# Parsoa/SVDSS

Hardware: AMD Instinct MI355X
Metric: reads/sec through search+call, 30x HiFi 15 kb reads vs 3 Gb ref, 1/2/4/8 GPU (higher is better)
Workload: dtype int64

## Files before the change

include/svdss_hip.h:

```cpp
#ifndef SVDSS_HIP_H
#define SVDSS_HIP_H

#include <stdint.h>

#ifdef __cplusplus
extern "C" {
#endif

#define SVDSS_OK 0
#define SVDSS_EINVAL 1
#define SVDSS_ENOMEM 2
#define SVDSS_EIO 3
#define SVDSS_EHIP 4
#define SVDSS_ENODEV 5
#define SVDSS_ERANGE 6

const char* svdss_strerror(int code);
const char* svdss_last_hip_error(void);

int svdss_nt6_encode(const char* seq, int64_t n, uint8_t* out);

typedef struct svdss_index svdss_index_t;

int svdss_index_build(const uint8_t* contigs, const int64_t* lens, int32_t n_contigs,
// ... 326 lines not shown
int32_t svdss_ref_stream_tile_bytes(void);

int svdss_place_sfs_batch(svdss_ref_t* ref, const int32_t* tid, const int32_t* pos, const uint32_t* cigar,
                          const int64_t* cigar_off, const int32_t* sfs_qs, const int32_t* sfs_len, const int64_t* sfs_off,
                          int64_t n_aln, int32_t* out_count, int32_t* out, int64_t stats[4]);

int svdss_smooth_batch(svdss_ref_t* ref, const int32_t* tid, const int32_t* pos, const uint32_t* cigar,
                       const int64_t* cigar_off, const uint8_t* seq4, const int64_t* seq4_off, const uint8_t* qual,
                       const int64_t* qual_off, const int32_t* l_seq, const int64_t* cap_off, int64_t n,
                       uint8_t* out_seq4, uint8_t* out_qual, uint32_t* out_cigar, int32_t* out_ncig, int32_t* out_len,
                       int64_t* out_match_mismatch, uint8_t* out_ignore);

typedef struct svdss_aln_batch svdss_aln_batch_t;

int svdss_align_global_batch(const uint8_t* queries, const int64_t* q_off, const uint8_t* targets,
                             const int64_t* t_off, int64_t n_pairs, int32_t m, const int8_t* mat,
                             int32_t gapo, int32_t gape, int32_t gapo2, int32_t gape2, int32_t device,
                             svdss_aln_batch_t** out);
int64_t svdss_aln_batch_npairs(const svdss_aln_batch_t* b);
int64_t svdss_aln_batch_total_cigar(const svdss_aln_batch_t* b);
int64_t svdss_aln_batch_cells(const svdss_aln_batch_t* b);
double svdss_aln_batch_kernel_ms(const svdss_aln_batch_t* b);
int svdss_aln_batch_launch_info(const svdss_aln_batch_t* b, int64_t out[4]);
int svdss_aln_batch_fetch(const svdss_aln_batch_t* b, int32_t* scores, int64_t* n_cigar, uint32_t* cigar);
void svdss_aln_batch_free(svdss_aln_batch_t* b);

typedef struct svdss_poa_batch svdss_poa_batch_t;

int svdss_poa_consensus_batch(const uint8_t* seqs, const int64_t* seq_off, const int64_t* cluster_off,
                              int64_t n_clusters, int32_t device, svdss_poa_batch_t** out);
int64_t svdss_poa_batch_nclusters(const svdss_poa_batch_t* b);
int64_t svdss_poa_batch_total(const svdss_poa_batch_t* b);
int64_t svdss_poa_batch_cells(const svdss_poa_batch_t* b);
double svdss_poa_batch_kernel_ms(const svdss_poa_batch_t* b);
int64_t svdss_poa_batch_hbm(const svdss_poa_batch_t* b);
int64_t svdss_poa_batch_quad_back(const svdss_poa_batch_t* b);
int svdss_poa_quad_selftest(const int32_t* in, int32_t* out, int32_t device);
int svdss_poa_batch_fetch(const svdss_poa_batch_t* b, int64_t* cons_len, uint8_t* cons);
void svdss_poa_batch_free(svdss_poa_batch_t* b);

int svdss_indel_ratio_batch(const uint8_t* a, const int64_t* a_off, const uint8_t* b, const int64_t* b_off,
                            int64_t n_pairs, int32_t device, double* ratio_out, int64_t* lcs_out);
int32_t svdss_indel_ratio_last_kernel(void);

int svdss_call_side_stat(int32_t device, int64_t out[4]);

// ... 41 lines not shown
```

svdss_amd/_lib.py:

```python
import ctypes as C
import os

_HERE = os.path.dirname(os.path.abspath(__file__))
LIB_PATH = os.environ.get("SVDSS_LIB") or os.path.join(_HERE, "libsvdss_hip.so")

SVDSS_OK = 0
SVDSS_SFS_ASSEMBLE = 1
SVDSS_BAM_PUTATIVE = 0x100


class SvdssError(RuntimeError):
    def __init__(self, code, where):
        self.code = code
        msg = lib.svdss_strerror(code).decode()
        hip = lib.svdss_last_hip_error().decode()
        super().__init__(f"{where}: {msg} (code {code})" + (f" [{hip}]" if hip else ""))


def _load():
    if not os.path.exists(LIB_PATH):
        raise ImportError(
            f"{LIB_PATH} not found: build it with `python -c 'import __graft_entry__ as g; g.build()'` "
            "or `make -C svdss_amd/csrc` (hipcc, gfx950). There is no CPU fallback."
        )
# ... 136 lines not shown
    "svdss_fastx_tile_bytes": (_i32, []),
    "svdss_ref_upload": (C.c_int, [_p, _p, _i32, _i32, C.POINTER(_p)]),
    "svdss_ref_upload_parts": (C.c_int, [_p, _p, _i32, _i32, C.POINTER(_p)]),
    "svdss_ref_free": (None, [_p]),
    "svdss_ref_read": (C.c_int, [_p, _pi32, _p, _p]),
    "svdss_ref_stream_create": (C.c_int, [_i32, _i64, C.POINTER(_p)]),
    "svdss_ref_stream_batch": (C.c_int, [_p, _i64, _i32, _i32, _p, _p, _p, _p, _p, _p, _i64]),
    "svdss_ref_stream_result": (C.c_int, [_p, _p]),
    "svdss_ref_stream_download": (C.c_int, [_p, _i64, _p]),
    "svdss_ref_stream_finish": (C.c_int, [_p, _p, _i32, _i32, C.POINTER(_p)]),
    "svdss_ref_stream_drop_host": (None, [_p]),
    "svdss_ref_stream_free": (None, [_p]),
    "svdss_ref_stream_error": (C.c_char_p, [_p]),
    "svdss_ref_stream_tile_bytes": (_i32, []),
    "svdss_place_sfs_batch": (C.c_int, [_p, _p, _p, _p, _p, _p, _p, _p, _i64, _p, _p, _p]),
    "svdss_smooth_batch": (C.c_int, [_p] * 11 + [_i64] + [_p] * 7),
    "svdss_align_global_batch": (C.c_int, [_p, _p, _p, _p, _i64, _i32, _p, _i32, _i32, _i32, _i32, _i32,
                                           C.POINTER(_p)]),
    "svdss_aln_batch_npairs": (_i64, [_p]),
    "svdss_aln_batch_total_cigar": (_i64, [_p]),
    "svdss_aln_batch_cells": (_i64, [_p]),
    "svdss_aln_batch_kernel_ms": (C.c_double, [_p]),
    "svdss_aln_batch_launch_info": (C.c_int, [_p, _p]),
    "svdss_aln_batch_fetch": (C.c_int, [_p, _p, _p, _p]),
    "svdss_aln_batch_free": (None, [_p]),
    "svdss_poa_consensus_batch": (C.c_int, [_p, _p, _p, _i64, _i32, C.POINTER(_p)]),
    "svdss_poa_batch_nclusters": (_i64, [_p]),
    "svdss_poa_batch_total": (_i64, [_p]),
    "svdss_poa_batch_cells": (_i64, [_p]),
    "svdss_poa_batch_kernel_ms": (C.c_double, [_p]),
    "svdss_poa_batch_hbm": (_i64, [_p]),
    "svdss_poa_batch_quad_back": (_i64, [_p]),
    "svdss_poa_quad_selftest": (C.c_int, [_p, _p, C.c_int32]),
    "svdss_poa_batch_fetch": (C.c_int, [_p, _p, _p]),
    "svdss_poa_batch_free": (None, [_p]),
    "svdss_indel_ratio_batch": (C.c_int, [_p, _p, _p, _p, _i64, _i32, _p, _p]),
    "svdss_indel_ratio_last_kernel": (_i32, []),
    "svdss_call_side_stat": (C.c_int, [_i32, _p]),
    "svdss_gzip_stream_create": (C.c_int, [_i32, _i64, C.POINTER(_p)]),
    "svdss_gzip_stream_run": (C.c_int, [_p, _p, _i64, _i32, _pi64]),
    "svdss_gzip_stream_result": (C.c_int, [_p, _p]),
    "svdss_gzip_stream_host_tail": (C.c_int, [_p, _p, _i64]),
    "svdss_gzip_stream_error": (C.c_char_p, [_p]),
    "svdss_gzip_stream_free": (None, [_p]),
}

# ... 10 lines not shown
```

svdss_amd/csrc/call_dp.hip:

```cpp
#include <hip/hip_runtime.h>

#include <cstdint>
#include <algorithm>
#include <chrono>
#include <cstdio>
#include <cstring>
#include <new>
#include <string>
#include <vector>

#include "../../include/svdss_hip.h"
#include "call_streams.h"
#include "dev_arena.h"
#include "hip_check.h"

#define DP_NEG (-0x20000000)
#define DP_THREADS 256

struct GapModel { int q, e, q2, e2; };

__device__ __forceinline__ int dp_gap(int l, const GapModel& g) {
  const int a = g.q + l * g.e, b = g.q2 + l * g.e2;
  return a < b ? a : b;
}

struct AlnPair {
  int64_t q_off, t_off;
  int64_t bnd_off;
  int64_t dir_off;
  int64_t cig_off;
  int32_t ql, tl;
  int32_t slot;
  int32_t waves;
};

__device__ __forceinline__ int dp_shr1(int x) {
  return __builtin_amdgcn_update_dpp(x, x, 0x138, 0xf, 0xf, false);
}

template <int W>
__global__ void __launch_bounds__(64 * W) align_wave_kernel(
    const AlnPair* pairs, const uint8_t* qsyms, const uint8_t* tsyms, int m, const int8_t* mat_g,
    GapModel gm, int32_t* ws, uint8_t* dirs, uint32_t* cigars, int32_t* scores, int32_t* n_cigar, int32_t* abort_flag) {
  const AlnPair P = pairs[blockIdx.x];
  const int ql = P.ql, tl = P.tl;
  const int lane = threadIdx.x & 63, wave = threadIdx.x >> 6;
  const int Wp = W > 1 ? P.waves : 1, NB = Wp + 1;
  if (wave >= Wp) return;
  if (ql <= 0 || tl <= 0) {
    if (lane == 0) { scores[P.slot] = 0; n_cigar[P.slot] = 0; }
    return;
  }
  __shared__ volatile int32_t prog[W + 1];
  __shared__ int32_t s_score;
  const uint8_t* q = qsyms + P.q_off;
  const uint8_t* t = tsyms + P.t_off;
  uint8_t* dir = dirs + P.dir_off;
  const int bstride = ql + 64;
  int32_t* bnd = ws + P.bnd_off;
  {
    int32_t* b0 = bnd + (int64_t)(NB - 1) * 3 * bstride;
    for (int j = threadIdx.x; j < ql; j += 64 * Wp) { b0[j] = -dp_gap(j + 1, gm); b0[bstride + j] = DP_NEG; b0[2 * bstride + j] = DP_NEG; }
    if ((int)threadIdx.x < NB) prog[threadIdx.x] = (int)threadIdx.x == NB - 1 ? ql : 0;
    __builtin_amdgcn_fence(__ATOMIC_RELEASE, "workgroup");
  }
  __syncthreads();
  const int n_stripes = (tl + 63) >> 6;
  int32_t final_score = 0;
  bool aborted = false;
  for (int s = wave; s < n_stripes && !aborted; s += Wp) {
    const int in_slot = (s + NB - 1) % NB, out_slot = s % NB;
    const int32_t* bin = bnd + (int64_t)in_slot * 3 * bstride;
    int32_t* bout = bnd + (int64_t)out_slot * 3 * bstride;
    if (W > 1 && lane == 0) prog[out_slot] = (s + 1) << 20;
    const int i = (s << 6) + lane;
    const bool row_ok = i < tl;
    const int rows = tl - (s << 6) < 64 ? tl - (s << 6) : 64;
    const bool writes_bnd = lane == 63 && s + 1 < n_stripes;
    uint64_t rowbits = 0;
    {
      const int ti = row_ok ? t[i] : 0;
      for (int k = 0; k < m; ++k) rowbits |= (uint64_t)(uint8_t)mat_g[ti * m + k] << (8 * k);
    }
    int32_t Hl = -dp_gap(i + 1, gm), Fl = DP_NEG, F2l = DP_NEG;
    int32_t Hout = 0, Eout = DP_NEG, E2out = DP_NEG;
    int32_t Hd = 0;
    int qcur = 0;
    const int n_steps = ql + rows - 1;
    int32_t nH = 0, nE = 0, nE2 = 0;
    int nq = 0;
    auto fetch = [&](int tau0) {
      const int jj = tau0 + lane;
      const bool in = jj < ql;
      nq = in ? q[jj] : 0;
      if (W > 1 && Wp > 1) {
        const int need = tau0 + 64 < ql ? tau0 + 64 : ql;
        int polls = 0;
        for (;;) {
          const int32_t v = prog[in_slot];
          if ((v >> 20) == s && (v & 0xFFFFF) >= need) break;
          if (++polls > (1 << 22)) { aborted = true; break; }
          __builtin_amdgcn_s_sleep(2);
        }
        if (aborted) { nH = 0; nE = 0; nE2 = 0; return; }
        __builtin_amdgcn_fence(__ATOMIC_ACQUIRE, "workgroup");
        nH = in ? __hip_atomic_load(&bin[jj], __ATOMIC_RELAXED, __HIP_MEMORY_SCOPE_WORKGROUP) : 0;
        nE = in ? __hip_atomic_load(&bin[bstride + jj], __ATOMIC_RELAXED, __HIP_MEMORY_SCOPE_WORKGROUP) : 0;
        nE2 = in ? __hip_atomic_load(&bin[2 * bstride + jj], __ATOMIC_RELAXED, __HIP_MEMORY_SCOPE_WORKGROUP) : 0;
      } else {
        nH = in ? bin[jj] : 0; nE = in ? bin[bstride + jj] : 0; nE2 = in ? bin[2 * bstride + jj] : 0;
      }
    };
    fetch(0);
    uint8_t* dcell = dir + (int64_t)(s << 6) * tl + i;
    for (int tau0 = 0; tau0 < n_steps && !aborted; tau0 += 64) {
      asm volatile("" : "+v"(nq), "+v"(nH), "+v"(nE), "+v"(nE2));
      const int qblk = nq;
      const int32_t bH = nH, bE = nE, bE2 = nE2;
      if (tau0 + 64 < n_steps) fetch(tau0 + 64);
      const int kmax = n_steps - tau0 < 64 ? n_steps - tau0 : 64;
      for (int k = 0; k < kmax; ++k) {
        const int tau = tau0 + k;
        const int qs = __builtin_amdgcn_readlane(qblk, k);
        const int32_t hb = __builtin_amdgcn_readlane(bH, k), eb = __builtin_amdgcn_readlane(bE, k),
                      e2b = __builtin_amdgcn_readlane(bE2, k);
        qcur = dp_shr1(qcur);
        int32_t Hu = dp_shr1(Hout), Eu = dp_shr1(Eout), E2u = dp_shr1(E2out);
        if (lane == 0) { qcur = qs; Hu = hb; Eu = eb; E2u = e2b; }
        const int j = tau - lane;
        if (row_ok && j >= 0 && j < ql) {
          const int32_t hdiag = j == 0 ? (i == 0 ? 0 : -dp_gap(i, gm)) : Hd;
          const int32_t Ein = (Hu - gm.q > Eu ? Hu - gm.q : Eu) - gm.e;
          const int32_t E2in = (Hu - gm.q2 > E2u ? Hu - gm.q2 : E2u) - gm.e2;
          const int32_t Fin = (Hl - gm.q > Fl ? Hl - gm.q : Fl) - gm.e;
          const int32_t F2in = (Hl - gm.q2 > F2l ? Hl - gm.q2 : F2l) - gm.e2;
          int32_t z = hdiag + (int32_t)(int8_t)(rowbits >> (8 * qcur));
          uint32_t d = 0;
          if (Ein > z) { d = 1; z = Ein; }
          if (Fin > z) { d = 2; z = Fin; }
          if (E2in > z) { d = 3; z = E2in; }
          if (F2in > z) { d = 4; z = F2in; }
          if (Ein > z - gm.q) d |= 0x08;
          if (Fin > z - gm.q) d |= 0x10;
          if (E2in > z - gm.q2) d |= 0x20;
          if (F2in > z - gm.q2) d |= 0x40;
          *dcell = (uint8_t)d;
          Hout = z; Eout = Ein; E2out = E2in;
          Hl = z; Fl = Fin; F2l = F2in;
          if (writes_bnd) { bout[j] = z; bout[bstride + j] = Ein; bout[2 * bstride + j] = E2in; }
          if (i == tl - 1 && j == ql - 1) final_score = z;
        }
        Hd = Hu;
        dcell += tl;
      }
      if (W > 1 && Wp > 1 && s + 1 < n_stripes) {
        __builtin_amdgcn_fence(__ATOMIC_RELEASE, "workgroup");
        const int done = tau0 + kmax - 63;
        if (lane == 63) prog[out_slot] = ((s + 1) << 20) | (done < 0 ? 0 : done > ql ? ql : done);
      }
    }
    if (W == 1 || Wp == 1) __syncthreads();
    else if (s + 1 < n_stripes) { __builtin_amdgcn_fence(__ATOMIC_RELEASE, "workgroup"); if (lane == 63) prog[out_slot] = ((s + 1) << 20) | ql; }
    if (s == n_stripes - 1) {
      const int owner = (tl - 1) & 63;
      final_score = __builtin_amdgcn_readlane(final_score, owner);
      if (lane == 0) s_score = final_score;
    }
  }
  if (aborted && lane == 0) atomicExch(abort_flag, 1);
  __syncthreads();
  if (wave != 0) return;
  final_score = s_score;
  {
    if (lane == 0) scores[P.slot] = final_score;
    uint32_t* cg = cigars + P.cig_off;
    int n = 0, i = tl - 1, j = ql - 1, state = 0;
    uint32_t cur_op = 0xffffffffu, cur_len = 0;
    auto push = [&](uint32_t op, uint32_t len) {
      if (op == cur_op) { cur_len += len; return; }
      if (cur_op != 0xffffffffu) { if (lane == 0) cg[n] = (cur_len << 4) | cur_op; ++n; }
      cur_op = op; cur_len = len;
    };
    int i0 = -(1 << 28), j0 = 0;
    uint32_t win = 0;
    while (i >= 0 && j >= 0) {
      int k = i0 - i, d = j - (j0 - k);
      if (k < 0 || k > 63 || d < 0 || d > 3) {
        i0 = i; j0 = j - 1; k = 0; d = 1;
        const int ii = i0 - lane;
        const int64_t jj = (int64_t)j0 - lane;
        win = 0;
        if (ii >= 0) {
#pragma unroll
          for (int x = 0; x < 4; ++x) {
            const int64_t c = jj + x;
            if (c >= 0 && c < ql) win |= (uint32_t)dir[(int64_t)(ii + c) * tl + ii] << (8 * x);
          }
        }
        asm volatile("" : "+v"(win));
      }
      const uint32_t tmp = ((uint32_t)__builtin_amdgcn_readlane((int)win, k) >> (8 * d)) & 0xffu;
      if (state == 0) state = tmp & 7;
      else if (!((tmp >> (state + 2)) & 1)) state = 0;
      if (state == 0) state = tmp & 7;
      if (state == 0) { push(0, 1); --i; --j; }
      else if (state == 1 || state == 3) { push(2, 1); --i; }
      else { push(1, 1); --j; }
    }
    if (i >= 0) push(2, (uint32_t)(i + 1));
    if (j >= 0) push(1, (uint32_t)(j + 1));
    if (cur_op != 0xffffffffu) { if (lane == 0) cg[n] = (cur_len << 4) | cur_op; ++n; }
    if (lane == 0) n_cigar[P.slot] = n;
  }
}

__device__ __forceinline__ void dp_lds_barrier() {
  __builtin_amdgcn_fence(__ATOMIC_RELEASE, "workgroup", "local");
  __builtin_amdgcn_s_barrier();
  __builtin_amdgcn_fence(__ATOMIC_ACQUIRE, "workgroup", "local");
}

struct LcsPair {
  int64_t a_off, b_off, ws_off;
  int32_t la, lb;
};

template <bool LDS>
__global__ void __launch_bounds__(DP_THREADS) lcs_ratio_kernel(const LcsPair* pairs, const uint8_t* as,
                                                              const uint8_t* bs, int32_t* ws,
                                                              int64_t* lcs_out, double* ratio_out) {
  extern __shared__ int32_t dp_lds[];
  const LcsPair P = pairs[blockIdx.x];
  const int la = P.la, lb = P.lb;
  int64_t lcs = 0;
  if (la > 0 && lb > 0) {
    const uint8_t* a = as + P.a_off;
// ... 79 lines not shown
    const int valid = m - 64 * lane;
    const unsigned long long vm = valid >= 64 ? ~0ull : valid <= 0 ? 0ull : ((1ull << valid) - 1);
    int z = (int)__popcll(~V & vm);
    for (int o = 32; o > 0; o >>= 1) z += __shfl_xor(z, o, 64);
    lcs = z;
  }
  if (lane == 0) {
    const int64_t maximum = (int64_t)P.la + P.lb;
    const int64_t dist = maximum - 2 * lcs;
    const double norm_dist = maximum ? (double)dist / (double)maximum : 0.0;
    const double norm_sim = 1.0 - norm_dist;
    lcs_out[blockIdx.x] = lcs;
    ratio_out[blockIdx.x] = norm_sim * 100.0;
  }
}


struct svdss_aln_batch {
  int64_t n_pairs = 0;
  int64_t total_cigar = 0;
  int64_t cells = 0;
  double kernel_ms = 0.0;
  int64_t info[4] = {0, 0, 0, 0};
  std::vector<int32_t> scores;
  std::vector<int64_t> n_cigar;
  std::vector<uint32_t> cigar;
  int device = -1;
  DevArena arena;
};

namespace {
struct DevMem {
  void* p = nullptr;
  ~DevMem() { if (p) (void)hipFree(p); }
  int alloc(size_t bytes) {
    HIPCHK(hipMalloc(&p, bytes ? bytes : 16));
    return SVDSS_OK;
  }
};
}

extern "C" int svdss_align_global_batch(const uint8_t* queries, const int64_t* q_off,
                                        const uint8_t* targets, const int64_t* t_off, int64_t n_pairs,
                                        int32_t m, const int8_t* mat, int32_t gapo, int32_t gape,
                                        int32_t gapo2, int32_t gape2, int32_t device,
                                        svdss_aln_batch_t** out) {
  if (!out || n_pairs < 0 || m < 1 || m > 8 || !mat || device < 0) return SVDSS_EINVAL;
  if (n_pairs > 0 && (!queries || !q_off || !targets || !t_off)) return SVDSS_EINVAL;
  HIPCHK(hipSetDevice(device));
  svdss_aln_batch* b = *out ? *out : new (std::nothrow) svdss_aln_batch();
  if (!b) return SVDSS_ENOMEM;
  *out = b;
  b->n_pairs = n_pairs;
  b->total_cigar = 0;
  b->cells = 0;
  b->kernel_ms = 0.0;
  b->info[0] = b->info[1] = b->info[2] = b->info[3] = 0;
  b->scores.assign((size_t)n_pairs, 0);
  b->n_cigar.assign((size_t)n_pairs, 0);
  b->cigar.clear();
  if (n_pairs == 0) return SVDSS_OK;
  for (int64_t i = 0; i < n_pairs; ++i) {
    const int64_t ql = q_off[i + 1] - q_off[i], tl = t_off[i + 1] - t_off[i];
    if (ql < 0 || tl < 0) return SVDSS_EINVAL;
    if (ql >= (1 << 28) || tl >= (1 << 28)) return SVDSS_ERANGE;
  }
  const int64_t qtot = q_off[n_pairs] - q_off[0], ttot = t_off[n_pairs] - t_off[0];
  if (b->device != device) {
    b->arena.drop();
    b->device = device;
  }
  CallStreamLease lease;
  HIPCHK(lease.acquire(device));
  const hipStream_t st = lease.get();
  const GapModel gm{gapo, gape, gapo2, gape2};
  hipEvent_t ev0, ev1;
  HIPCHK(hipEventCreate(&ev0));
  HIPCHK(hipEventCreate(&ev1));
  int64_t dir_budget = (int64_t)24 << 30;
  {
    size_t free_b = 0, total_b = 0;
    if (hipMemGetInfo(&free_b, &total_b) == hipSuccess)
      dir_budget = std::min<int64_t>(dir_budget, (int64_t)((free_b + b->arena.cap) / 2));
    if (dir_budget < ((int64_t)1 << 30)) dir_budget = (int64_t)1 << 30;
    if (getenv("SVDSS_ALIGN_DIR_MB") && atoll(getenv("SVDSS_ALIGN_DIR_MB")) > 0) dir_budget = atoll(getenv("SVDSS_ALIGN_DIR_MB")) << 20;
  }
  std::vector<int32_t> h_nc((size_t)n_pairs, 0);
  std::vector<std::pair<int64_t, int64_t>> cig_at((size_t)n_pairs);
  std::vector<std::vector<uint32_t>> chunk_cigs;
  int64_t start = 0;
  const int ALN_W = getenv("SVDSS_ALIGN_WAVES") && atoi(getenv("SVDSS_ALIGN_WAVES")) == 8 ? 8 : 4;
  const int64_t aln_frac = getenv("SVDSS_ALIGN_FRAC") && atoll(getenv("SVDSS_ALIGN_FRAC")) > 0 ? atoll(getenv("SVDSS_ALIGN_FRAC")) : 8;
  int64_t max_cells = 0;
  for (int64_t i = 0; i < n_pairs; ++i) max_cells = std::max(max_cells, (q_off[i + 1] - q_off[i]) * (t_off[i + 1] - t_off[i]));
  bool multi = !(getenv("SVDSS_ALIGN_WAVES") && atoi(getenv("SVDSS_ALIGN_WAVES")) <= 1);
  auto waves_of = [&](int64_t ql, int64_t tl) {
    if (!multi || tl < 8 * 64 || ql >= (1 << 20)) return 1;
    return (ql * tl * aln_frac >= max_cells || n_pairs < 2048) ? ALN_W : 1;
  };
  while (start < n_pairs) {
    std::vector<AlnPair> hp;
    int64_t ws = 0, dirb = 0, cig = 0, end = start;
    bool any_multi = false;
    while (end < n_pairs) {
      const int64_t ql = q_off[end + 1] - q_off[end], tl = t_off[end + 1] - t_off[end];
      const int64_t need = (ql + tl) * tl;
      if (end > start && dirb + need > dir_budget) break;
      AlnPair a;
      memset(&a, 0, sizeof a);
      a.q_off = q_off[end] - q_off[0];
      a.t_off = t_off[end] - t_off[0];
      a.bnd_off = ws;
      a.dir_off = dirb;
      a.cig_off = cig;
      a.ql = (int32_t)ql;
      a.tl = (int32_t)tl;
      a.slot = (int32_t)(end - start);
      a.waves = waves_of(ql, tl);
      any_multi = any_multi || a.waves > 1;
      hp.push_back(a);
      cig_at[(size_t)end] = {cig, (int64_t)chunk_cigs.size()};
      ws += 3 * (a.waves + 1) * (ql + 64);
      dirb += need;
      cig += ql + tl + 2;
      b->cells += ql * tl;
      ++end;
    }
    const int64_t np = end - start;
    std::stable_sort(hp.begin(), hp.end(), [](const AlnPair& x, const AlnPair& y) {
      return (int64_t)x.ql * x.tl > (int64_t)y.ql * y.tl;
    });
    const size_t need_bytes = DevArena::padded((size_t)qtot) + DevArena::padded((size_t)ttot) + DevArena::padded(64) +
                              DevArena::padded(sizeof(AlnPair) * (size_t)np) + DevArena::padded(sizeof(int32_t) * (size_t)ws) +
                              DevArena::padded((size_t)dirb) + DevArena::padded(sizeof(uint32_t) * (size_t)cig) +
                              2 * DevArena::padded(sizeof(int32_t) * (size_t)np) + DevArena::padded(64);
    HIPCHK(b->arena.reserve(need_bytes));
    void* d_q = b->arena.take((size_t)qtot);
    void* d_t = b->arena.take((size_t)ttot);
    void* d_mat = b->arena.take(64);
    void* d_pairs = b->arena.take(sizeof(AlnPair) * (size_t)np);
    void* d_ws = b->arena.take(sizeof(int32_t) * (size_t)ws);
    void* d_dir = b->arena.take((size_t)dirb);
    void* d_cig = b->arena.take(sizeof(uint32_t) * (size_t)cig);
    void* d_sc = b->arena.take(sizeof(int32_t) * (size_t)np);
    void* d_nc = b->arena.take(sizeof(int32_t) * (size_t)np);
    void* d_abort = b->arena.take(64);
    if (qtot) HIPCHK(hipMemcpyAsync(d_q, queries + q_off[0], (size_t)qtot, hipMemcpyHostToDevice, st));
    if (ttot) HIPCHK(hipMemcpyAsync(d_t, targets + t_off[0], (size_t)ttot, hipMemcpyHostToDevice, st));
    HIPCHK(hipMemcpyAsync(d_mat, mat, (size_t)(m * m), hipMemcpyHostToDevice, st));
    HIPCHK(hipMemcpyAsync(d_pairs, hp.data(), sizeof(AlnPair) * (size_t)np, hipMemcpyHostToDevice, st));
    HIPCHK(hipMemsetAsync(d_abort, 0, 64, st));
    HIPCHK(hipEventRecord(ev0, st));
    if (any_multi && ALN_W == 8)
      hipLaunchKernelGGL(align_wave_kernel<8>, dim3((unsigned)np), dim3(64 * 8), 0, st, (const AlnPair*)d_pairs,
                         (const uint8_t*)d_q, (const uint8_t*)d_t, (int)m, (const int8_t*)d_mat, gm, (int32_t*)d_ws,
                         (uint8_t*)d_dir, (uint32_t*)d_cig, (int32_t*)d_sc, (int32_t*)d_nc, (int32_t*)d_abort);
    else if (any_multi)
      hipLaunchKernelGGL(align_wave_kernel<4>, dim3((unsigned)np), dim3(64 * 4), 0, st, (const AlnPair*)d_pairs,
                         (const uint8_t*)d_q, (const uint8_t*)d_t, (int)m, (const int8_t*)d_mat, gm, (int32_t*)d_ws,
                         (uint8_t*)d_dir, (uint32_t*)d_cig, (int32_t*)d_sc, (int32_t*)d_nc, (int32_t*)d_abort);
    else
      hipLaunchKernelGGL(align_wave_kernel<1>, dim3((unsigned)np), dim3(64), 0, st, (const AlnPair*)d_pairs,
                         (const uint8_t*)d_q, (const uint8_t*)d_t, (int)m, (const int8_t*)d_mat, gm, (int32_t*)d_ws,
                         (uint8_t*)d_dir, (uint32_t*)d_cig, (int32_t*)d_sc, (int32_t*)d_nc, (int32_t*)d_abort);
    HIPCHK(hipGetLastError());
    HIPCHK(hipEventRecord(ev1, st));
    if (any_multi) {
      int32_t ab = 0;
      HIPCHK(hipMemcpyAsync(&ab, d_abort, sizeof ab, hipMemcpyDeviceToHost, st));
      HIPCHK(hipStreamSynchronize(st));
      if (ab) {
        fprintf(stderr, "[svdss] realignment: a multi-wavefront pair did not finish; the batch runs again with one wavefront per pair\n");
        multi = false;
        ++b->info[3];
        b->cells -= [&] { int64_t c = 0; for (const AlnPair& a : hp) c += (int64_t)a.ql * a.tl; return c; }();
        for (int64_t k = start; k < end; ++k) cig_at[(size_t)k] = {0, 0};
        continue;
      }
    }
    ++b->info[0];
    for (const AlnPair& a : hp) b->info[1] += a.waves > 1;
    b->info[2] = std::max<int64_t>(b->info[2], any_multi ? ALN_W : 1);
    chunk_cigs.emplace_back((size_t)cig);
    HIPCHK(hipMemcpyAsync(&b->scores[(size_t)start], d_sc, sizeof(int32_t) * (size_t)np, hipMemcpyDeviceToHost, st));
    HIPCHK(hipMemcpyAsync(&h_nc[(size_t)start], d_nc, sizeof(int32_t) * (size_t)np, hipMemcpyDeviceToHost, st));
    if (cig) HIPCHK(hipMemcpyAsync(chunk_cigs.back().data(), d_cig, sizeof(uint32_t) * (size_t)cig, hipMemcpyDeviceToHost, st));
    HIPCHK(hipStreamSynchronize(st));
    float ms = 0.f;
    HIPCHK(hipEventElapsedTime(&ms, ev0, ev1));
    b->kernel_ms += ms;
    start = end;
  }
  {
    int64_t total = 0;
    for (int64_t k = 0; k < n_pairs; ++k) total += h_nc[(size_t)k];
    b->cigar.resize((size_t)total);
    int64_t o = 0;
    for (int64_t k = 0; k < n_pairs; ++k) {
      const int32_t nc = h_nc[(size_t)k];
      b->n_cigar[(size_t)k] = nc;
      const uint32_t* src = chunk_cigs[(size_t)cig_at[(size_t)k].second].data() + cig_at[(size_t)k].first;
      for (int x = nc - 1; x >= 0; --x) b->cigar[(size_t)o++] = src[x];
    }
  }
  (void)hipEventDestroy(ev0);
  (void)hipEventDestroy(ev1);
  b->total_cigar = (int64_t)b->cigar.size();
  return SVDSS_OK;
}

extern "C" int64_t svdss_aln_batch_npairs(const svdss_aln_batch_t* b) { return b ? b->n_pairs : -1; }
extern "C" int64_t svdss_aln_batch_total_cigar(const svdss_aln_batch_t* b) { return b ? b->total_cigar : -1; }
extern "C" int64_t svdss_aln_batch_cells(const svdss_aln_batch_t* b) { return b ? b->cells : -1; }
extern "C" double svdss_aln_batch_kernel_ms(const svdss_aln_batch_t* b) { return b ? b->kernel_ms : -1.0; }

extern "C" int svdss_aln_batch_launch_info(const svdss_aln_batch_t* b, int64_t out[4]) {
  if (!b || !out) return SVDSS_EINVAL;
  memcpy(out, b->info, sizeof b->info);
  return SVDSS_OK;
}

extern "C" int svdss_aln_batch_fetch(const svdss_aln_batch_t* b, int32_t* scores, int64_t* n_cigar,
                                     uint32_t* cigar) {
  if (!b) return SVDSS_EINVAL;
  if (scores) memcpy(scores, b->scores.data(), sizeof(int32_t) * b->scores.size());
  if (n_cigar) memcpy(n_cigar, b->n_cigar.data(), sizeof(int64_t) * b->n_cigar.size());
  if (cigar) memcpy(cigar, b->cigar.data(), sizeof(uint32_t) * b->cigar.size());
  return SVDSS_OK;
}

extern "C" void svdss_aln_batch_free(svdss_aln_batch_t* b) { delete b; }

static thread_local int32_t g_ratio_last_kernel = -1;
extern "C" int32_t svdss_indel_ratio_last_kernel(void) { return g_ratio_last_kernel; }

extern "C" int svdss_indel_ratio_batch(const uint8_t* a, const int64_t* a_off, const uint8_t* bsy,
                                       const int64_t* b_off, int64_t n_pairs, int32_t device,
                                       double* ratio_out, int64_t* lcs_out) {
  if (n_pairs < 0 || device < 0) return SVDSS_EINVAL;
  if (n_pairs == 0) return SVDSS_OK;
  if (!a || !a_off || !bsy || !b_off || !ratio_out) return SVDSS_EINVAL;
// ... 91 lines not shown
```

Measured before the change: 8.414 million.

## Add provable score-bound banding to global realignment DP kernel

Computes a score lower bound per pair on the GPU (best single-gap alignment) and uses it to derive a provable diagonal band, optionally with a carried dead zone between two bands. The wavefront DP then skips stripe steps outside the band and carries gap state across the skipped region, and traceback handles the skipped region too. The goal is to cut DP cells for long, similar realignment pairs. Input uploads also move out of the per-chunk loop into a separate arena. The cost is an extra kernel plus a host sync per batch, more workspace, and considerably more complex control flow that risks correctness bugs.

```diff
diff --git a/include/svdss_hip.h b/include/svdss_hip.h
--- a/include/svdss_hip.h
+++ b/include/svdss_hip.h
@@ -372,6 +372,7 @@
 int64_t svdss_aln_batch_cells(const svdss_aln_batch_t* b);
 double svdss_aln_batch_kernel_ms(const svdss_aln_batch_t* b);
 int svdss_aln_batch_launch_info(const svdss_aln_batch_t* b, int64_t out[4]);
+int svdss_aln_batch_band_info(const svdss_aln_batch_t* b, int64_t out[4]);
 int svdss_aln_batch_fetch(const svdss_aln_batch_t* b, int32_t* scores, int64_t* n_cigar, uint32_t* cigar);
 void svdss_aln_batch_free(svdss_aln_batch_t* b);
 
diff --git a/svdss_amd/_lib.py b/svdss_amd/_lib.py
--- a/svdss_amd/_lib.py
+++ b/svdss_amd/_lib.py
@@ -182,6 +182,7 @@
     "svdss_aln_batch_cells": (_i64, [_p]),
     "svdss_aln_batch_kernel_ms": (C.c_double, [_p]),
     "svdss_aln_batch_launch_info": (C.c_int, [_p, _p]),
+    "svdss_aln_batch_band_info": (C.c_int, [_p, _p]),
     "svdss_aln_batch_fetch": (C.c_int, [_p, _p, _p, _p]),
     "svdss_aln_batch_free": (None, [_p]),
     "svdss_poa_consensus_batch": (C.c_int, [_p, _p, _p, _i64, _i32, C.POINTER(_p)]),
diff --git a/svdss_amd/csrc/aln_band.h b/svdss_amd/csrc/aln_band.h
--- /dev/null
+++ b/svdss_amd/csrc/aln_band.h
@@ -0,0 +1,150 @@
+#pragma once
+#include <cstddef>
+#include <cstdint>
+#include <vector>
+
+#ifdef __HIPCC__
+#define ALN_HD __host__ __device__
+#else
+#define ALN_HD
+#endif
+
+#define ALN_BAND_MIN_DEAD 128
+
+enum { ALN_FULL = 0, ALN_ONE_BAND = 1, ALN_CARRY = 2 };
+
+struct AlnBand {
+  int32_t lo, hi, c1, c2;
+  int32_t mode;
+};
+
+struct AlnScoring {
+  int m;
+  const int8_t* mat;
+  int q, e, q2, e2;
+};
+
+inline int64_t aln_gap(int64_t k, const AlnScoring& s) {
+  if (k <= 0) return 0;
+  const int64_t a = s.q + k * s.e, b = s.q2 + k * s.e2;
+  return a < b ? a : b;
+}
+
+inline AlnBand aln_band_full(int64_t ql, int64_t tl) {
+  AlnBand b;
+  b.lo = (int32_t)-tl;
+  b.hi = (int32_t)ql;
+  b.c1 = b.hi;
+  b.c2 = b.hi + 1;
+  b.mode = ALN_FULL;
+  return b;
+}
+
+inline bool aln_band_provable(const AlnScoring& s, int* M_out) {
+  int M = -128;
+  for (int k = 0; k < s.m * s.m; ++k) M = s.mat[k] > M ? s.mat[k] : M;
+  *M_out = M;
+  return M > 0 && s.q >= 0 && s.e >= 0 && s.q2 >= 0 && s.e2 >= 0;
+}
+
+inline int64_t aln_band_f(int64_t d, int64_t ql, int64_t tl, int M, const AlnScoring& s) {
+  const int64_t D = ql - tl;
+  return (int64_t)M * (ql < tl ? ql : tl) - aln_gap(d < 0 ? -d : d, s) - aln_gap(D - d < 0 ? d - D : D - d, s);
+}
+
+inline int64_t aln_band_slb(const uint8_t* q, int64_t ql, const uint8_t* t, int64_t tl, const AlnScoring& s, int64_t* x_out,
+                            std::vector<int32_t>& pre) {
+  const int64_t n = ql < tl ? ql : tl, D = ql - tl, k = D < 0 ? -D : D;
+  const int64_t qs = D > 0 ? D : 0, ts = D < 0 ? -D : 0;
+  pre.resize((size_t)n + 1);
+  int32_t acc = 0;
+  pre[0] = 0;
+  for (int64_t x = 0; x < n; ++x) { acc += s.mat[t[x] * s.m + q[x]]; pre[(size_t)x + 1] = acc; }
+  if (D == 0) { *x_out = 0; return acc; }
+  int64_t best = pre[(size_t)n], best_x = n;
+  int32_t suf = 0;
+  for (int64_t x = n - 1; x >= 0; --x) {
+    suf += s.mat[t[x + ts] * s.m + q[x + qs]];
+    const int64_t v = (int64_t)pre[(size_t)x] + suf;
+    if (v >= best) { best = v; best_x = x; }
+  }
+  *x_out = best_x;
+  return best - aln_gap(k, s);
+}
+
+inline AlnBand aln_band_plan_slb(int64_t ql, int64_t tl, const AlnScoring& s, int level, int64_t slb) {
+  AlnBand b = aln_band_full(ql, tl);
+  int M = 0;
+  if (level <= 0 || ql <= 0 || tl <= 0 || !aln_band_provable(s, &M)) return b;
+  const int64_t D = ql - tl;
+  const int64_t h0 = D < 0 ? D : 0, h1 = D < 0 ? 0 : D;
+  auto f = [&](int64_t d) { return aln_band_f(d, ql, tl, M, s); };
+  int64_t lo = h0, hi = h1, c1 = h0, c2 = h1;
+  while (lo - 1 >= -tl && f(lo - 1) >= slb) --lo;
+  while (hi + 1 <= ql && f(hi + 1) >= slb) ++hi;
+  while (c1 + 1 < h1 && f(c1 + 1) >= slb) ++c1;
+  while (c2 - 1 > c1 && f(c2 - 1) >= slb) --c2;
+  b.lo = (int32_t)lo;
+  b.hi = (int32_t)hi;
+  if (level >= 2 && c2 - c1 - 1 >= ALN_BAND_MIN_DEAD) {
+    b.c1 = (int32_t)c1;
+    b.c2 = (int32_t)c2;
+    b.mode = ALN_CARRY;
+  } else {
+    b.c1 = b.hi;
+    b.c2 = b.hi + 1;
+    b.mode = ALN_ONE_BAND;
+  }
+  return b;
+}
+
+inline AlnBand aln_band_plan(const uint8_t* q, int64_t ql, const uint8_t* t, int64_t tl, const AlnScoring& s, int level,
+                             std::vector<int32_t>& scratch, int64_t* slb_out = nullptr, int64_t* x_out = nullptr) {
+  int M = 0;
+  int64_t x = 0, slb = 0;
+  if (level > 0 && ql > 0 && tl > 0 && aln_band_provable(s, &M)) slb = aln_band_slb(q, ql, t, tl, s, &x, scratch);
+  if (slb_out) *slb_out = slb;
+  if (x_out) *x_out = x;
+  return aln_band_plan_slb(ql, tl, s, level, slb);
+}
+
+ALN_HD inline bool aln_band_live(int d, const AlnBand& b) {
+  return (unsigned)(d - b.lo) <= (unsigned)(b.hi - b.lo) && !((unsigned)(d - b.c1 - 1) < (unsigned)(b.c2 - b.c1 - 1));
+}
+
+struct AlnStripeSteps { int a[2], e[2]; };
+ALN_HD inline AlnStripeSteps aln_band_stripe_steps(int ql, int tl, int s, const AlnBand& b) {
+  const int i0 = s << 6, rows = tl - i0 < 64 ? tl - i0 : 64, n_steps = ql + rows - 1;
+  AlnStripeSteps r;
+  r.a[1] = r.e[1] = n_steps;
+  if (b.mode == ALN_FULL) { r.a[0] = 0; r.e[0] = n_steps; return r; }
+  const int64_t spread = 2 * (rows - 1) + 1;
+  const bool two = b.mode == ALN_CARRY;
+  int64_t a0 = (int64_t)b.lo + i0, e0 = (int64_t)(two ? b.c1 : b.hi) + i0 + spread;
+  a0 = a0 < 0 ? 0 : a0 & ~(int64_t)63;
+  e0 = e0 < 0 ? 0 : e0 > n_steps ? n_steps : e0;
+  if (a0 > e0) a0 = e0;
+  r.a[0] = (int)a0; r.e[0] = (int)e0;
+  if (two) {
+    int64_t a1 = (int64_t)b.c2 + i0, e1 = (int64_t)b.hi + i0 + spread;
+    a1 = a1 < 0 ? 0 : a1 & ~(int64_t)63;
+    if (e1 > n_steps) e1 = n_steps;
+    if (a1 < e1) {
+      if (a1 < e0 + 2) r.e[0] = (int)e1;
+      else { r.a[1] = (int)a1; r.e[1] = (int)e1; }
+    }
+  }
+  return r;
+}
+
+inline int64_t aln_band_steps(int64_t ql, int64_t tl, const AlnBand& b, int64_t* full_out = nullptr) {
+  int64_t steps = 0, full = 0;
+  if (ql > 0 && tl > 0)
+    for (int s = 0; s < (int)((tl + 63) >> 6); ++s) {
+      const AlnStripeSteps r = aln_band_stripe_steps((int)ql, (int)tl, s, b);
+      steps += (r.e[0] - r.a[0]) + (r.e[1] - r.a[1]);
+      full += ql + (tl - 64 * (int64_t)s < 64 ? tl - 64 * (int64_t)s : 64) - 1;
+    }
+  if (full_out) *full_out = full;
+  return steps;
+}
diff --git a/svdss_amd/csrc/call_dp.hip b/svdss_amd/csrc/call_dp.hip
--- a/svdss_amd/csrc/call_dp.hip
+++ b/svdss_amd/csrc/call_dp.hip
@@ -10,6 +10,7 @@
 #include <vector>
 
 #include "../../include/svdss_hip.h"
+#include "aln_band.h"
 #include "call_streams.h"
 #include "dev_arena.h"
 #include "hip_check.h"
@@ -32,25 +33,20 @@
   int32_t ql, tl;
   int32_t slot;
   int32_t waves;
+  AlnBand band;
 };
 
 __device__ __forceinline__ int dp_shr1(int x) {
   return __builtin_amdgcn_update_dpp(x, x, 0x138, 0xf, 0xf, false);
 }
 
-template <int W>
-__global__ void __launch_bounds__(64 * W) align_wave_kernel(
-    const AlnPair* pairs, const uint8_t* qsyms, const uint8_t* tsyms, int m, const int8_t* mat_g,
-    GapModel gm, int32_t* ws, uint8_t* dirs, uint32_t* cigars, int32_t* scores, int32_t* n_cigar, int32_t* abort_flag) {
-  const AlnPair P = pairs[blockIdx.x];
+template <int W, bool BAND>
+__device__ __forceinline__ void align_pair(
+    const AlnPair& P, const uint8_t* qsyms, const uint8_t* tsyms, int m, const int8_t* mat_g,
+    const GapModel& gm, int32_t* ws, uint8_t* dirs, uint32_t* cigars, int32_t* scores, int32_t* n_cigar, int32_t* abort_flag) {
   const int ql = P.ql, tl = P.tl;
   const int lane = threadIdx.x & 63, wave = threadIdx.x >> 6;
   const int Wp = W > 1 ? P.waves : 1, NB = Wp + 1;
-  if (wave >= Wp) return;
-  if (ql <= 0 || tl <= 0) {
-    if (lane == 0) { scores[P.slot] = 0; n_cigar[P.slot] = 0; }
-    return;
-  }
   __shared__ volatile int32_t prog[W + 1];
   __shared__ int32_t s_score;
   const uint8_t* q = qsyms + P.q_off;
@@ -58,6 +54,14 @@
   uint8_t* dir = dirs + P.dir_off;
   const int bstride = ql + 64;
   int32_t* bnd = ws + P.bnd_off;
+  const AlnBand B = P.band;
+  const bool horiz = BAND && B.mode == ALN_CARRY && ql > tl, vert = BAND && B.mode == ALN_CARRY && ql < tl;
+  const int dead_w = B.c2 - B.c1 - 1;
+  int32_t* xarr = bnd + (int64_t)NB * 3 * bstride;
+  auto decayed = [](int32_t v, int per, int n) {
+    const int64_t x = (int64_t)v - (int64_t)per * n;
+    return x < DP_NEG ? (int32_t)DP_NEG : (int32_t)x;
+  };
   {
     int32_t* b0 = bnd + (int64_t)(NB - 1) * 3 * bstride;
     for (int j = threadIdx.x; j < ql; j += 64 * Wp) { b0[j] = -dp_gap(j + 1, gm); b0[bstride + j] = DP_NEG; b0[2 * bstride + j] = DP_NEG; }
@@ -82,43 +86,78 @@
       const int ti = row_ok ? t[i] : 0;
       for (int k = 0; k < m; ++k) rowbits |= (uint64_t)(uint8_t)mat_g[ti * m + k] << (8 * k);
     }
-    int32_t Hl = -dp_gap(i + 1, gm), Fl = DP_NEG, F2l = DP_NEG;
+    int32_t Hl = !BAND || aln_band_live(-i, B) ? -dp_gap(i + 1, gm) : DP_NEG, Fl = DP_NEG, F2l = DP_NEG;
     int32_t Hout = 0, Eout = DP_NEG, E2out = DP_NEG;
     int32_t Hd = 0;
     int qcur = 0;
     const int n_steps = ql + rows - 1;
+    AlnStripeSteps R;
+    if (BAND) R = aln_band_stripe_steps(ql, tl, s, B);
+    else { R.a[0] = 0; R.e[0] = n_steps; R.a[1] = R.e[1] = n_steps; }
+    const int dl = (s << 6) + 2 * lane;
+    const int xcol = B.c1 + i;
+    int32_t Xv = DP_NEG, X2v = DP_NEG;
     int32_t nH = 0, nE = 0, nE2 = 0;
     int nq = 0;
+    const int32_t none = BAND ? DP_NEG : 0;
+    auto wait_above = [&](int need) {
+      int polls = 0;
+      for (;;) {
+        const int32_t v = prog[in_slot];
+        if ((v >> 20) == s && (v & 0xFFFFF) >= need) return;
+        if (++polls > (1 << 22)) { aborted = true; return; }
+        __builtin_amdgcn_s_sleep(2);
+      }
+    };
     auto fetch = [&](int tau0) {
       const int jj = tau0 + lane;
-      const bool in = jj < ql;
-      nq = in ? q[jj] : 0;
+      const bool in = jj < ql && (!BAND || aln_band_live(jj - (s << 6) + 1, B));
+      const bool xin = vert && row_ok && xcol >= 0 && xcol < ql && xcol + lane >= tau0 && xcol + lane < tau0 + 64;
+      nq = jj < ql ? q[jj] : 0;
       if (W > 1 && Wp > 1) {
-        const int need = tau0 + 64 < ql ? tau0 + 64 : ql;
-        int polls = 0;
-        for (;;) {
-          const int32_t v = prog[in_slot];
-          if ((v >> 20) == s && (v & 0xFFFFF) >= need) break;
-          if (++polls > (1 << 22)) { aborted = true; break; }
-          __builtin_amdgcn_s_sleep(2);
-        }
+        wait_above(tau0 + 64 < ql ? tau0 + 64 : ql);
         if (aborted) { nH = 0; nE = 0; nE2 = 0; return; }
         __builtin_amdgcn_fence(__ATOMIC_ACQUIRE, "workgroup");
-        nH = in ? __hip_atomic_load(&bin[jj], __ATOMIC_RELAXED, __HIP_MEMORY_SCOPE_WORKGROUP) : 0;
-        nE = in ? __hip_atomic_load(&bin[bstride + jj], __ATOMIC_RELAXED, __HIP_MEMORY_SCOPE_WORKGROUP) : 0;
-        nE2 = in ? __hip_atomic_load(&bin[2 * bstride + jj], __ATOMIC_RELAXED, __HIP_MEMORY_SCOPE_WORKGROUP) : 0;
+        nH = in ? __hip_atomic_load(&bin[jj], __ATOMIC_RELAXED, __HIP_MEMORY_SCOPE_WORKGROUP) : none;
+        nE = in ? __hip_atomic_load(&bin[bstride + jj], __ATOMIC_RELAXED, __HIP_MEMORY_SCOPE_WORKGROUP) : none;
+        nE2 = in ? __hip_atomic_load(&bin[2 * bstride + jj], __ATOMIC_RELAXED, __HIP_MEMORY_SCOPE_WORKGROUP) : none;
+        if (BAND && xin) {
+          Xv = decayed(__hip_atomic_load(&xarr[xcol], __ATOMIC_RELAXED, __HIP_MEMORY_SCOPE_WORKGROUP), gm.e, dead_w);
+          X2v = decayed(__hip_atomic_load(&xarr[bstride + xcol], __ATOMIC_RELAXED, __HIP_MEMORY_SCOPE_WORKGROUP), gm.e2, dead_w);
+        }
       } else {
-        nH = in ? bin[jj] : 0; nE = in ? bin[bstride + jj] : 0; nE2 = in ? bin[2 * bstride + jj] : 0;
+        nH = in ? bin[jj] : none; nE = in ? bin[bstride + jj] : none; nE2 = in ? bin[2 * bstride + jj] : none;
+        if (BAND && xin) { Xv = decayed(xarr[xcol], gm.e, dead_w); X2v = decayed(xarr[bstride + xcol], gm.e2, dead_w); }
       }
     };
-    fetch(0);
-    uint8_t* dcell = dir + (int64_t)(s << 6) * tl + i;
-    for (int tau0 = 0; tau0 < n_steps && !aborted; tau0 += 64) {
+    for (int r = 0; r < (BAND ? 2 : 1) && !aborted; ++r) {
+    const int ra = r ? R.a[1] : R.a[0], re = r ? R.e[1] : R.e[0];
+    if (ra >= re) continue;
+    fetch(ra);
+    if (BAND && ra > 0 && !aborted) {
+      const int jq = ra - 1 - lane;
+      qcur = jq >= 0 && jq < ql ? q[jq] : 0;
+      Hout = DP_NEG; Eout = DP_NEG; E2out = DP_NEG;
+      Hd = DP_NEG;
+      if (lane == 0 && ra - 1 < ql && aln_band_live(ra - (s << 6), B))
+        Hd = W > 1 && Wp > 1 ? __hip_atomic_load(&bin[ra - 1], __ATOMIC_RELAXED, __HIP_MEMORY_SCOPE_WORKGROUP) : bin[ra - 1];
+      if (ra - lane > 0) {
+        if (horiz && r == 1) {
+          Fl = decayed(Hl - gm.q > Fl ? Hl - gm.q : Fl, gm.e, ra - R.e[0]);
+          F2l = decayed(Hl - gm.q2 > F2l ? Hl - gm.q2 : F2l, gm.e2, ra - R.e[0]);
+        }
+        else { Fl = DP_NEG; F2l = DP_NEG; }
+        Hl = DP_NEG;
+      }
+    }
+    uint8_t* dcell = dir + (int64_t)((s << 6) + ra) * tl + i;
+    for (int tau0 = ra; tau0 < re && !aborted; tau0 += 64) {
       asm volatile("" : "+v"(nq), "+v"(nH), "+v"(nE), "+v"(nE2));
+      if (BAND) asm volatile("" : "+v"(Xv), "+v"(X2v));
       const int qblk = nq;
       const int32_t bH = nH, bE = nE, bE2 = nE2;
-      if (tau0 + 64 < n_steps) fetch(tau0 + 64);
-      const int kmax = n_steps - tau0 < 64 ? n_steps - tau0 : 64;
+      if (tau0 + 64 < re) fetch(tau0 + 64);
+      const int kmax = re - tau0 < 64 ? re - tau0 : 64;
       for (int k = 0; k < kmax; ++k) {
         const int tau = tau0 + k;
         const int qs = __builtin_amdgcn_readlane(qblk, k);
@@ -128,10 +167,20 @@
         int32_t Hu = dp_shr1(Hout), Eu = dp_shr1(Eout), E2u = dp_shr1(E2out);
         if (lane == 0) { qcur = qs; Hu = hb; Eu = eb; E2u = e2b; }
         const int j = tau - lane;
-        if (row_ok && j >= 0 && j < ql) {
+        const bool inr = row_ok && j >= 0 && j < ql;
+        const int dg = tau - dl;
+        if (BAND && inr && !aln_band_live(dg, B)) {
+          if (horiz && dg > B.c1 && dg < B.c2) {
+            Fl = (Hl - gm.q > Fl ? Hl - gm.q : Fl) - gm.e;
+            F2l = (Hl - gm.q2 > F2l ? Hl - gm.q2 : F2l) - gm.e2;
+          } else { Fl = DP_NEG; F2l = DP_NEG; }
+          Hl = DP_NEG;
+          Hout = DP_NEG; Eout = DP_NEG; E2out = DP_NEG;
+        } else if (inr) {
           const int32_t hdiag = j == 0 ? (i == 0 ? 0 : -dp_gap(i, gm)) : Hd;
-          const int32_t Ein = (Hu - gm.q > Eu ? Hu - gm.q : Eu) - gm.e;
-          const int32_t E2in = (Hu - gm.q2 > E2u ? Hu - gm.q2 : E2u) - gm.e2;
+          int32_t Ein = (Hu - gm.q > Eu ? Hu - gm.q : Eu) - gm.e;
+          int32_t E2in = (Hu - gm.q2 > E2u ? Hu - gm.q2 : E2u) - gm.e2;
+          if (BAND && vert && dg == B.c1) { Ein = Xv; E2in = X2v; }
           const int32_t Fin = (Hl - gm.q > Fl ? Hl - gm.q : Fl) - gm.e;
           const int32_t F2in = (Hl - gm.q2 > F2l ? Hl - gm.q2 : F2l) - gm.e2;
           int32_t z = hdiag + (int32_t)(int8_t)(rowbits >> (8 * qcur));
@@ -148,6 +197,10 @@
           Hout = z; Eout = Ein; E2out = E2in;
           Hl = z; Fl = Fin; F2l = F2in;
           if (writes_bnd) { bout[j] = z; bout[bstride + j] = Ein; bout[2 * bstride + j] = E2in; }
+          if (BAND && vert && dg == B.c2) {
+            xarr[j] = (z - gm.q > Ein ? z - gm.q : Ein) - gm.e;
+            xarr[bstride + j] = (z - gm.q2 > E2in ? z - gm.q2 : E2in) - gm.e2;
+          }
           if (i == tl - 1 && j == ql - 1) final_score = z;
         }
         Hd = Hu;
@@ -159,8 +212,13 @@
         if (lane == 63) prog[out_slot] = ((s + 1) << 20) | (done < 0 ? 0 : done > ql ? ql : done);
       }
     }
+    }
     if (W == 1 || Wp == 1) __syncthreads();
-    else if (s + 1 < n_stripes) { __builtin_amdgcn_fence(__ATOMIC_RELEASE, "workgroup"); if (lane == 63) prog[out_slot] = ((s + 1) << 20) | ql; }
+    else if (s + 1 < n_stripes) {
+      if (BAND && vert && !aborted) { wait_above(ql); __builtin_amdgcn_fence(__ATOMIC_ACQUIRE, "workgroup"); }
+      __builtin_amdgcn_fence(__ATOMIC_RELEASE, "workgroup");
+      if (lane == 63) prog[out_slot] = ((s + 1) << 20) | ql;
+    }
     if (s == n_stripes - 1) {
       const int owner = (tl - 1) & 63;
       final_score = __builtin_amdgcn_readlane(final_score, owner);
@@ -184,6 +242,15 @@
     int i0 = -(1 << 28), j0 = 0;
     uint32_t win = 0;
     while (i >= 0 && j >= 0) {
+      if (BAND && !aln_band_live(j - i, B)) {
+        const int dg = j - i;
+        if (horiz && dg > B.c1 && dg < B.c2 && (state == 2 || state == 4)) { push(1, (uint32_t)(dg - B.c1)); j -= dg - B.c1; }
+        else if (vert && dg > B.c1 && dg < B.c2 && (state == 1 || state == 3)) { push(2, (uint32_t)(B.c2 - dg)); i -= B.c2 - dg; }
+        else if (state == 0) { push(0, 1); --i; --j; }
+        else if (state == 1 || state == 3) { push(2, 1); --i; }
+        else { push(1, 1); --j; }
+        continue;
+      }
       int k = i0 - i, d = j - (j0 - k);
       if (k < 0 || k > 63 || d < 0 || d > 3) {
         i0 = i; j0 = j - 1; k = 0; d = 1;
@@ -212,6 +279,58 @@
     if (cur_op != 0xffffffffu) { if (lane == 0) cg[n] = (cur_len << 4) | cur_op; ++n; }
     if (lane == 0) n_cigar[P.slot] = n;
   }
+}
+
+template <int W>
+__global__ void __launch_bounds__(64 * W) align_wave_kernel(
+    const AlnPair* pairs, const uint8_t* qsyms, const uint8_t* tsyms, int m, const int8_t* mat_g,
+    GapModel gm, int32_t* ws, uint8_t* dirs, uint32_t* cigars, int32_t* scores, int32_t* n_cigar, int32_t* abort_flag) {
+  const AlnPair P = pairs[blockIdx.x];
+  if ((int)(threadIdx.x >> 6) >= (W > 1 ? P.waves : 1)) return;
+  if (P.ql <= 0 || P.tl <= 0) {
+    if ((threadIdx.x & 63) == 0) { scores[P.slot] = 0; n_cigar[P.slot] = 0; }
+    return;
+  }
+  if (P.band.mode != ALN_FULL) align_pair<W, true>(P, qsyms, tsyms, m, mat_g, gm, ws, dirs, cigars, scores, n_cigar, abort_flag);
+  else align_pair<W, false>(P, qsyms, tsyms, m, mat_g, gm, ws, dirs, cigars, scores, n_cigar, abort_flag);
+}
+
+__global__ void __launch_bounds__(64) aln_slb_kernel(const uint8_t* qsyms, const int64_t* q_off, const uint8_t* tsyms, const int64_t* t_off,
+                                                     int m, const int8_t* mat_g, int64_t* sum_out, int32_t* bad) {
+  const int64_t p = blockIdx.x;
+  const int64_t ql = q_off[p + 1] - q_off[p], tl = t_off[p + 1] - t_off[p];
+  const int64_t n = ql < tl ? ql : tl, D = ql - tl;
+  const int lane = threadIdx.x;
+  if (n <= 0) { if (lane == 0) sum_out[p] = 0; return; }
+  const uint8_t* q = qsyms + (q_off[p] - q_off[0]);
+  const uint8_t* t = tsyms + (t_off[p] - t_off[0]);
+  const int64_t qs = D > 0 ? D : 0, ts = D < 0 ? -D : 0;
+  const int64_t per = (n + 63) >> 6, k0 = lane * per, k1 = k0 + per < n ? k0 + per : n;
+  bool off = false;
+  auto score = [&](int tsym, int qsym) {
+    if (tsym >= m || qsym >= m) { off = true; return 0; }
+    return (int)mat_g[tsym * m + qsym];
+  };
+  int64_t sb = 0, sc = 0, mp = 0;
+  for (int64_t k = k0; k < k1; ++k) {
+    const int a = score(t[k], q[k]), bq = D != 0 ? score(t[k + ts], q[k + qs]) : a;
+    sb += bq;
+    sc += a - bq;
+    mp = sc > mp ? sc : mp;
+  }
+  if (__any(off) && lane == 0) atomicExch(bad, 1);
+  int64_t before = sc;
+  for (int o = 1; o < 64; o <<= 1) {
+    const int64_t v = __shfl_up(before, o, 64);
+    if (lane >= o) before += v;
+  }
+  int64_t best = before - sc + mp, tot = sb;
+  for (int o = 32; o > 0; o >>= 1) {
+    const int64_t v = __shfl_xor(best, o, 64), w = __shfl_xor(tot, o, 64);
+    best = v > best ? v : best;
+    tot += w;
+  }
+  if (lane == 0) sum_out[p] = tot + (best > 0 ? best : 0);
 }
 
 __device__ __forceinline__ void dp_lds_barrier() {
@@ -337,11 +456,13 @@
   int64_t cells = 0;
   double kernel_ms = 0.0;
   int64_t info[4] = {0, 0, 0, 0};
+  int64_t band[4] = {0, 0, 0, 0};
   std::vector<int32_t> scores;
   std::vector<int64_t> n_cigar;
   std::vector<uint32_t> cigar;
   int device = -1;
   DevArena arena;
+  DevArena in_arena;
 };
 
 namespace {
@@ -371,6 +492,7 @@
   b->cells = 0;
   b->kernel_ms = 0.0;
   b->info[0] = b->info[1] = b->info[2] = b->info[3] = 0;
+  b->band[0] = b->band[1] = b->band[2] = b->band[3] = 0;
   b->scores.assign((size_t)n_pairs, 0);
   b->n_cigar.assign((size_t)n_pairs, 0);
   b->cigar.clear();
@@ -383,6 +505,7 @@
   const int64_t qtot = q_off[n_pairs] - q_off[0], ttot = t_off[n_pairs] - t_off[0];
   if (b->device != device) {
     b->arena.drop();
+    b->in_arena.drop();
     b->device = device;
   }
   CallStreamLease lease;
@@ -413,6 +536,46 @@
     if (!multi || tl < 8 * 64 || ql >= (1 << 20)) return 1;
     return (ql * tl * aln_frac >= max_cells || n_pairs < 2048) ? ALN_W : 1;
   };
+  HIPCHK(b->in_arena.reserve(DevArena::padded((size_t)qtot) + DevArena::padded((size_t)ttot) + DevArena::padded(64) +
+                             3 * DevArena::padded(sizeof(int64_t) * (size_t)(n_pairs + 1)) + DevArena::padded(64)));
+  void* d_q = b->in_arena.take((size_t)qtot);
+  void* d_t = b->in_arena.take((size_t)ttot);
+  void* d_mat = b->in_arena.take(64);
+  if (qtot) HIPCHK(hipMemcpyAsync(d_q, queries + q_off[0], (size_t)qtot, hipMemcpyHostToDevice, st));
+  if (ttot) HIPCHK(hipMemcpyAsync(d_t, targets + t_off[0], (size_t)ttot, hipMemcpyHostToDevice, st));
+  HIPCHK(hipMemcpyAsync(d_mat, mat, (size_t)(m * m), hipMemcpyHostToDevice, st));
+  int band_level = getenv("SVDSS_ALIGN_BAND") ? std::max(0, std::min(2, atoi(getenv("SVDSS_ALIGN_BAND")))) : 2;
+  std::vector<AlnBand> bands((size_t)n_pairs);
+  std::vector<int64_t> band_steps((size_t)n_pairs), full_steps((size_t)n_pairs);
+  {
+    const AlnScoring sc{(int)m, mat, gapo, gape, gapo2, gape2};
+    int M = 0;
+    std::vector<int64_t> sums((size_t)n_pairs, 0);
+    if (band_level > 0 && aln_band_provable(sc, &M)) {
+      void* d_qo = b->in_arena.take(sizeof(int64_t) * (size_t)(n_pairs + 1));
+      void* d_to = b->in_arena.take(sizeof(int64_t) * (size_t)(n_pairs + 1));
+      void* d_sum = b->in_arena.take(sizeof(int64_t) * (size_t)n_pairs);
+      void* d_bad = b->in_arena.take(64);
+      int32_t bad = 0;
+      HIPCHK(hipMemcpyAsync(d_qo, q_off, sizeof(int64_t) * (size_t)(n_pairs + 1), hipMemcpyHostToDevice, st));
+      HIPCHK(hipMemcpyAsync(d_to, t_off, sizeof(int64_t) * (size_t)(n_pairs + 1), hipMemcpyHostToDevice, st));
+      HIPCHK(hipMemsetAsync(d_bad, 0, 64, st));
+      hipLaunchKernelGGL(aln_slb_kernel, dim3((unsigned)n_pairs), dim3(64), 0, st, (const uint8_t*)d_q, (const int64_t*)d_qo,
+                         (const uint8_t*)d_t, (const int64_t*)d_to, (int)m, (const int8_t*)d_mat, (int64_t*)d_sum, (int32_t*)d_bad);
+      HIPCHK(hipGetLastError());
+      HIPCHK(hipMemcpyAsync(sums.data(), d_sum, sizeof(int64_t) * (size_t)n_pairs, hipMemcpyDeviceToHost, st));
+      HIPCHK(hipMemcpyAsync(&bad, d_bad, sizeof bad, hipMemcpyDeviceToHost, st));
+      HIPCHK(hipStreamSynchronize(st));
+      if (bad) band_level = 0;
+    } else {
+      band_level = 0;
+    }
+    for (int64_t i = 0; i < n_pairs; ++i) {
+      const int64_t ql = q_off[i + 1] - q_off[i], tl = t_off[i + 1] - t_off[i], k = ql < tl ? tl - ql : ql - tl;
+      bands[(size_t)i] = aln_band_plan_slb(ql, tl, sc, band_level, sums[(size_t)i] - aln_gap(k, sc));
+      band_steps[(size_t)i] = aln_band_steps(ql, tl, bands[(size_t)i], &full_steps[(size_t)i]);
+    }
+  }
   while (start < n_pairs) {
     std::vector<AlnPair> hp;
     int64_t ws = 0, dirb = 0, cig = 0, end = start;
@@ -432,27 +595,24 @@
       a.tl = (int32_t)tl;
       a.slot = (int32_t)(end - start);
       a.waves = waves_of(ql, tl);
+      a.band = bands[(size_t)end];
       any_multi = any_multi || a.waves > 1;
       hp.push_back(a);
       cig_at[(size_t)end] = {cig, (int64_t)chunk_cigs.size()};
-      ws += 3 * (a.waves + 1) * (ql + 64);
+      ws += (3 * (a.waves + 1) + 2) * (ql + 64);
       dirb += need;
       cig += ql + tl + 2;
       b->cells += ql * tl;
       ++end;
     }
     const int64_t np = end - start;
-    std::stable_sort(hp.begin(), hp.end(), [](const AlnPair& x, const AlnPair& y) {
-      return (int64_t)x.ql * x.tl > (int64_t)y.ql * y.tl;
+    std::stable_sort(hp.begin(), hp.end(), [&](const AlnPair& x, const AlnPair& y) {
+      return band_steps[(size_t)(start + x.slot)] > band_steps[(size_t)(start + y.slot)];
     });
-    const size_t need_bytes = DevArena::padded((size_t)qtot) + DevArena::padded((size_t)ttot) + DevArena::padded(64) +
-                              DevArena::padded(sizeof(AlnPair) * (size_t)np) + DevArena::padded(sizeof(int32_t) * (size_t)ws) +
+    const size_t need_bytes = DevArena::padded(sizeof(AlnPair) * (size_t)np) + DevArena::padded(sizeof(int32_t) * (size_t)ws) +
                               DevArena::padded((size_t)dirb) + DevArena::padded(sizeof(uint32_t) * (size_t)cig) +
                               2 * DevArena::padded(sizeof(int32_t) * (size_t)np) + DevArena::padded(64);
     HIPCHK(b->arena.reserve(need_bytes));
-    void* d_q = b->arena.take((size_t)qtot);
-    void* d_t = b->arena.take((size_t)ttot);
-    void* d_mat = b->arena.take(64);
     void* d_pairs = b->arena.take(sizeof(AlnPair) * (size_t)np);
     void* d_ws = b->arena.take(sizeof(int32_t) * (size_t)ws);
     void* d_dir = b->arena.take((size_t)dirb);
@@ -460,9 +620,6 @@
     void* d_sc = b->arena.take(sizeof(int32_t) * (size_t)np);
     void* d_nc = b->arena.take(sizeof(int32_t) * (size_t)np);
     void* d_abort = b->arena.take(64);
-    if (qtot) HIPCHK(hipMemcpyAsync(d_q, queries + q_off[0], (size_t)qtot, hipMemcpyHostToDevice, st));
-    if (ttot) HIPCHK(hipMemcpyAsync(d_t, targets + t_off[0], (size_t)ttot, hipMemcpyHostToDevice, st));
-    HIPCHK(hipMemcpyAsync(d_mat, mat, (size_t)(m * m), hipMemcpyHostToDevice, st));
     HIPCHK(hipMemcpyAsync(d_pairs, hp.data(), sizeof(AlnPair) * (size_t)np, hipMemcpyHostToDevice, st));
     HIPCHK(hipMemsetAsync(d_abort, 0, 64, st));
     HIPCHK(hipEventRecord(ev0, st));
@@ -494,7 +651,13 @@
       }
     }
     ++b->info[0];
-    for (const AlnPair& a : hp) b->info[1] += a.waves > 1;
+    for (const AlnPair& a : hp) {
+      b->info[1] += a.waves > 1;
+      b->band[0] += band_steps[(size_t)(start + a.slot)];
+      b->band[1] += full_steps[(size_t)(start + a.slot)];
+      b->band[2] += a.band.mode == ALN_ONE_BAND;
+      b->band[3] += a.band.mode == ALN_CARRY;
+    }
     b->info[2] = std::max<int64_t>(b->info[2], any_multi ? ALN_W : 1);
     chunk_cigs.emplace_back((size_t)cig);
     HIPCHK(hipMemcpyAsync(&b->scores[(size_t)start], d_sc, sizeof(int32_t) * (size_t)np, hipMemcpyDeviceToHost, st));
@@ -532,6 +695,12 @@
 extern "C" int svdss_aln_batch_launch_info(const svdss_aln_batch_t* b, int64_t out[4]) {
   if (!b || !out) return SVDSS_EINVAL;
   memcpy(out, b->info, sizeof b->info);
+  return SVDSS_OK;
+}
+
+extern "C" int svdss_aln_batch_band_info(const svdss_aln_batch_t* b, int64_t out[4]) {
+  if (!b || !out) return SVDSS_EINVAL;
+  memcpy(out, b->band, sizeof b->band);
   return SVDSS_OK;
 }
 
```

After: 8.943 million, median of 6. 1.06x the previous value.
